# jgaeddert/liquid-usrp

Measured on AMD Instinct MI355X. Metric: complex Msamples/s through multichannelrx, higher is better.
Workload: dtype f32

## Files before the change

liquid-usrp_amd/csrc/channelizer.hip:

```cpp
#include "devel.h"
#include "devmath.h"
#include "kernels.h"
#include "sc16.hpp"
#include "devscope.hpp"

namespace mcrx {

#ifndef CH_NT_STORE
#define CH_NT_STORE 1
#endif
#ifndef CH_NT_LOAD
#define CH_NT_LOAD 1
#endif
#define CH_R 8
static_assert(MCRX_TILE_S == 2 * CH_R, "two rounds fill one granule");
#define CH_P_REF 14
#ifndef CH_RH
#define CH_RH 4
#endif
#define CH_P_OVS 28

__device__ __forceinline__ void lds_barrier()
{
    asm volatile("s_waitcnt lgkmcnt(0)\n\ts_barrier" ::: "memory");
// ... 4 lines not shown

template <int K> struct Log2 { enum { v = 1 + Log2<K / 2>::v }; };
template <> struct Log2<1> { enum { v = 0 }; };

#ifndef CH_RADIX8
#define CH_RADIX8 1
#endif
template <int K> struct Plan {
    enum { R = (CH_RADIX8 && (K == 1024 || K == 512)) ? 8 : 4, LR = R == 8 ? 3 : 2 };
    static constexpr int stages() { int L = K, s = 0; while (L > 16) { L /= R; s++; } return s; }
    static constexpr int final_size() { int L = K; while (L > 16) L /= R; return L; }
    enum { S = stages(), F = final_size(), RL = K + K / F, ROWP = RL + 1 };
};
template <int K> __device__ __forceinline__ int pad(int e) { return e + e / Plan<K>::F; }
template <int K>
__device__ __forceinline__ int dif_pos(int k)
{
    int L = K, pos = 0;
#pragma unroll
    for (int s = 0; s < Plan<K>::S; s++) { pos += (k & (Plan<K>::R - 1)) * (L >> Plan<K>::LR); k >>= Plan<K>::LR; L >>= Plan<K>::LR; }
    return pos + k;
}

__device__ __forceinline__ float2 w16(int k)
{
    const float c[8] = { 1.0f, 0.92387953251f, 0.70710678119f, 0.38268343236f, 0.0f, -0.38268343236f, -0.70710678119f, -0.92387953251f };
    const float s[8] = { 0.0f, -0.38268343236f, -0.70710678119f, -0.92387953251f, -1.0f, -0.92387953251f, -0.70710678119f, -0.38268343236f };
    return make_float2(c[k], s[k]);
}
constexpr int bitrev_c(int i, int bits) { int r = 0; for (int b = 0; b < bits; b++) if (i & (1 << b)) r |= 1 << (bits - 1 - b); return r; }

template <int F, bool LOWER = false>
__device__ __forceinline__ void fft_reg(float2 (&v)[F])
{
#pragma unroll
    for (int h = F / 2; h >= 1; h >>= 1) {
#pragma unroll
        for (int i = 0; i < F; i++) {
            if ((i & h) == 0) {
                const float2 u = v[i], w = v[i + h];
                v[i] = cadd(u, w);
                if (LOWER && h == 1) continue;
                const float2 d = csub(u, w);
                const int tk = (i & (h - 1)) * (8 / h);
                if (tk == 0) v[i + h] = d;
                else if (tk == 4) v[i + h] = cmulnj(d);
                else v[i + h] = cmul_fx(d, w16(tk));
            }
        }
    }
}

template <int K, int C, int T, int P> struct Geo {
    enum { TPS = K / C, NS = T / TPS, TILE_F2 = NS * CH_R * Plan<K>::ROWP };
    static constexpr int taps_in_lds() { const long room = (160l * 1024 - (long)TILE_F2 * 8) / (4l * K); return room >= P ? P : (int)room; }
    enum { TL = taps_in_lds() };
    static constexpr size_t lds_bytes() { return (size_t)TILE_F2 * sizeof(float2) + (size_t)TL * K * sizeof(float); }
};

template <int K, int C, int T, int P, bool SHIFT, int IN, bool EDGE>
__device__ __forceinline__ void channelizer_rounds(const ChanArgs &a, float2 *tile)
{
    typedef typename RawOf<IN>::type Raw;
    constexpr bool SC16 = IN == IQ_SC16;
    constexpr int TPS = K / C;
    constexpr int NS = T / TPS;
    constexpr int N = K / 2;
    constexpr int H = P - 1;
    constexpr int TL = Geo<K, C, T, P>::TL, TG = P - TL;
    constexpr int S = Plan<K>::S, F = Plan<K>::F, ROWP = Plan<K>::ROWP, R = Plan<K>::R, LR = Plan<K>::LR;
    static_assert(TPS * C == K && NS * TPS == T && NS >= 1, "bad channelizer geometry");
    static_assert(TL >= 1 && TG >= 0 && TG <= 8, "tap split");

    const int tid = threadIdx.x;
    const int sl = tid / TPS, cg = tid % TPS;
    const int n0 = cg * C;
    const long long slab = (long long)blockIdx.x * NS + sl;
    const long long bs = slab * (long long)a.slab_blocks;

    float *ltap = reinterpret_cast<float *>(tile + NS * CH_R * ROWP);
    {
        constexpr int NT = TL * K;
        constexpr int PER = (NT + T - 1) / T;
        float tv[PER];
#pragma unroll
        for (int i = 0; i < PER; i++) { const int idx = tid + i * T; tv[i] = a.taps[idx < NT ? idx : 0]; }
#pragma unroll
        for (int i = 0; i < PER; i++) { const int idx = tid + i * T; if (idx < NT) ltap[idx] = tv[i]; }
    }
    __syncthreads();
    float2 tw[S > 0 ? S : 1][R - 1];
#pragma unroll
    for (int st = 0; st < S; st++) {
        const int L = K >> (LR * st), q4 = L >> LR;
        const int pos = tid % q4;
#pragma unroll
        for (int r = 1; r < R; r++) {
            float sn, cs; sincos_u32((uint32_t)(r * pos) * (uint32_t)(4294967296.0 / L), sn, cs);
            tw[st][r - 1] = make_float2(cs, -sn);
        }
    }

    const uint32_t dth = a.dtheta;
    float sd1, cd1; sincos_u32(dth, sd1, cd1);
    float sk8, ck8; sincos_u32((uint32_t)K * dth, sk8, ck8);
    const uint32_t t0 = a.first_sample_lo;

    const Raw *const xin = static_cast<const Raw *>(a.x), *const hin = static_cast<const Raw *>(a.halo);
    auto load_raw = [&](long long b, Raw (&dst)[C]) {
        const Raw *src = xin + n0;
        if constexpr (EDGE) {
            const bool inx = b >= 0 && b < (long long)a.nblocks;
            const bool inh = b < 0 && hin != nullptr;
            if (inx) src = xin + (size_t)b * K + n0;
            if (inh) src = hin + (size_t)(b + H) * K + n0;
        } else if constexpr (SC16) src = xin + (uint32_t)((uint32_t)b * (uint32_t)K + (uint32_t)n0);
        else src = xin + (size_t)b * K + n0;
        if constexpr (SC16) {
            if constexpr (C == 2) {
#if CH_NT_LOAD
                typedef uint32_t v2u __attribute__((ext_vector_type(2)));
                const v2u v = __builtin_nontemporal_load(reinterpret_cast<const v2u *>(src));
#else
                const uint2 v = *reinterpret_cast<const uint2 *>(src);
#endif
                dst[0] = v.x; dst[1] = v.y;
            } else dst[0] = src[0];
        } else if constexpr (C == 2) {
#if CH_NT_LOAD
            typedef float v4f __attribute__((ext_vector_type(4)));
            const v4f v = __builtin_nontemporal_load(reinterpret_cast<const v4f *>(src));
#else
            const float4 v = *reinterpret_cast<const float4 *>(src);
#endif
            dst[0] = make_float2(v.x, v.y); dst[1] = make_float2(v.z, v.w);
        } else dst[0] = src[0];
    };
    auto osc_start = [&](long long g, float &sn, float &cs) {
        sincos_u32_hw((t0 + (uint32_t)(g * K + n0)) * dth, sn, cs);
    };
    auto osc_next_block = [&](float &sn, float &cs) {
        const float s2 = fmaf(sn, ck8, cs * sk8), c2 = fmaf(cs, ck8, -(sn * sk8)); sn = s2; cs = c2;
    };
    auto mix_with = [&](long long b, float sn, float cs, const Raw (&src)[C], float2 (&dst)[C]) {
        if constexpr (EDGE) {
            const bool valid = (b >= 0 && b < (long long)a.nblocks) || (b < 0 && a.halo != nullptr);
            sn = valid ? sn : 0.f; cs = valid ? cs : 0.f;
        }
#pragma unroll
        for (int c = 0; c < C; c++) {
            if (c > 0) { const float s2 = fmaf(sn, cd1, cs * sd1), c2 = fmaf(cs, cd1, -(sn * sd1)); sn = s2; cs = c2; }
            float x, y;
            if constexpr (SC16) { x = (float)(int16_t)(src[c] & 0xffffu) * 0x1p-15f; y = (float)((int32_t)src[c] >> 16) * 0x1p-15f; }
            else { x = src[c].x; y = src[c].y; }
            dst[c] = make_float2(fmaf(x, cs, y * sn), fmaf(y, cs, -(x * sn)));
        }
    };

    float2 s[H + CH_R][C];
    Raw w[SC16 ? H + CH_R : 1][C];
    auto raw = [&](int i) -> Raw (&)[C] { if constexpr (SC16) return w[i]; else return s[i]; };
#pragma unroll
    for (int i = 0; i < H + CH_R; i++) load_raw(bs - H + i, raw(i));
    {
        constexpr int HG = (H + CH_R - 1) / CH_R, HSKIP = HG * CH_R - H;
        static_assert(CH_R == 8, "groups of 8");
        int i = 0;
#pragma unroll
        for (int g = 0; g < HG; g++) {
            float sn, cs;
            osc_start(bs - (long long)CH_R * (HG - g), sn, cs);
#pragma unroll
            for (int k = 0; k < CH_R; k++) {
                if (g > 0 || k >= HSKIP) { mix_with(bs - H + i, sn, cs, raw(i), s[i]); i++; }
                osc_next_block(sn, cs);
            }
        }
    }

    constexpr int NBF4 = NS * CH_R * (K / R);
    constexpr int NG = NS * CH_R * (K / F);
    constexpr int NOPS = NS * N * (CH_R / 2);
    static_assert(S == 0 || (NBF4 % T == 0 && T % (K / R) == 0), "a thread's butterflies must differ by whole rows");
    static_assert(NG % T == 0 || NG < T, "F-point groups per thread");
    static_assert(NOPS % T == 0, "granule stores per thread");
    constexpr int BTRIPS = S > 0 ? NBF4 / T : 0, BSTEP = S > 0 ? (T / (K / R)) * ROWP : 0;
    int fa[S > 0 ? S : 1];
    if constexpr (S > 0) {
#pragma unroll
        for (int st = 0; st < S; st++) {
            const int L = K >> (LR * st), q4 = L >> LR;
            const int f = tid / (K / R), j = tid % (K / R);
            fa[st] = f * ROWP + pad<K>((j / q4) * L + j % q4);
        }
    }
    constexpr int GTRIPS = (NG + T - 1) / T;
    int fg[GTRIPS];
#pragma unroll
    for (int i = 0; i < GTRIPS; i++) { const int g = tid + i * T; fg[i] = (g / (K / F)) * ROWP + (g % (K / F)) * (F + 1); }
    constexpr int OTRIPS = NOPS / T;
    int ssrc[OTRIPS];
    uint32_t sdst[OTRIPS];
    int srem[OTRIPS];
#pragma unroll
    for (int k = 0; k < OTRIPS; k++) {
        const int o = tid + k * T;
        const int osl = o / (N * (CH_R / 2)), rem = o % (N * (CH_R / 2));
        const int ch = rem / (CH_R / 2), rp = rem % (CH_R / 2);
        const long long ob = ((long long)blockIdx.x * NS + osl) * (long long)a.slab_blocks;
        const int g = ch / a.cg, c = ch % a.cg;
        ssrc[k] = (osl * CH_R + 2 * rp) * ROWP + pad<K>(dif_pos<K>(ch));
        sdst[k] = (uint32_t)((((size_t)g * a.ntiles + (size_t)(ob / MCRX_TILE_S)) * a.cg + c) * (MCRX_TILE_S / 2) + rp);
        const long long left = (long long)a.nblocks - ob;
        srem[k] = left < 0 ? 0 : (left > 0x40000000ll ? 0x40000000 : (int)left);
    }
    const uint32_t tile_step = a.cg * (MCRX_TILE_S / 2);
    float4 *out4 = reinterpret_cast<float4 *>(a.out);
    int wcol[C];
#pragma unroll
    for (int c = 0; c < C; c++) wcol[c] = pad<K>(SHIFT ? (int)((n0 + c + a.col_shift) & (K - 1)) : n0 + c);

    const int rounds = a.slab_blocks / CH_R;
    for (int rd = 0; rd < rounds; rd++) {
        const long long b0 = bs + (long long)rd * CH_R;
        float tg[TG > 0 ? TG : 1][C];
#pragma unroll
        for (int j = 0; j < TG; j++)
#pragma unroll
            for (int c = 0; c < C; c++) tg[j][c] = a.taps[(size_t)(TL + j) * K + n0 + c];
        if constexpr (P <= CH_P_REF) {
            float tap[P][C];
#pragma unroll
            for (int j = 0; j < P; j++)
#pragma unroll
                for (int c = 0; c < C; c++) tap[j][c] = ltap[j * K + n0 + c];
            {
                float sn, cs;
                osc_start(b0, sn, cs);
#pragma unroll
                for (int r = 0; r < CH_R; r++) { mix_with(b0 + r, sn, cs, raw(H + r), s[H + r]); osc_next_block(sn, cs); }
            }
#pragma unroll
            for (int r = 0; r < CH_R; r++) {
                float2 v[C];
#pragma unroll
                for (int c = 0; c < C; c++) v[c] = make_float2(0.f, 0.f);
#pragma unroll
                for (int j = P - 1; j >= 0; j--) {
#pragma unroll
                    for (int c = 0; c < C; c++) {
                        v[c].x += tap[j][c] * s[H + r - j][c].x;
                        v[c].y += tap[j][c] * s[H + r - j][c].y;
                    }
                }
                float2 *row = tile + (sl * CH_R + r) * ROWP;
                if constexpr (SHIFT) {
#pragma unroll
                    for (int c = 0; c < C; c++) row[wcol[c]] = v[c];
                } else {
                    float2 *rw = row + pad<K>(n0);
#pragma unroll
                    for (int c = 0; c < C; c++) rw[c] = v[c];
                }
            }
        } else {
            {
                float sn, cs;
                osc_start(b0, sn, cs);
#pragma unroll
                for (int r = 0; r < CH_R; r++) { mix_with(b0 + r, sn, cs, raw(H + r), s[H + r]); osc_next_block(sn, cs); }
            }
#pragma unroll
            for (int rh = 0; rh < CH_R; rh += CH_RH) {
                float2 v[CH_RH][C];
#pragma unroll
                for (int r = 0; r < CH_RH; r++)
#pragma unroll
                    for (int c = 0; c < C; c++) v[r][c] = make_float2(0.f, 0.f);
#pragma unroll
                for (int j = P - 1; j >= 0; j--) {
                    float tj[C];
#pragma unroll
                    for (int c = 0; c < C; c++) tj[c] = j >= TL ? tg[j - TL][c] : ltap[j * K + n0 + c];
#pragma unroll
                    for (int r = 0; r < CH_RH; r++)
#pragma unroll
                        for (int c = 0; c < C; c++) {
                            v[r][c].x += tj[c] * s[H + rh + r - j][c].x;
                            v[r][c].y += tj[c] * s[H + rh + r - j][c].y;
                        }
                }
#pragma unroll
                for (int r = 0; r < CH_RH; r++) {
// ... 12 lines not shown
#pragma unroll
        for (int i = 0; i < H; i++)
#pragma unroll
            for (int c = 0; c < C; c++) s[i][c] = s[i + CH_R][c];
#pragma unroll
        for (int r = 0; r < CH_R; r++) load_raw(b0 + CH_R + r, raw(H + r));
        lds_barrier();

        if constexpr (S > 0) {
#pragma unroll
            for (int st = 0; st < S; st++) {
                const int L = K >> (LR * st), q4 = L >> LR;
                const int D = q4 + q4 / F;
#pragma unroll
                for (int i = 0; i < BTRIPS; i++) {
                    float2 *p = tile + fa[st] + i * BSTEP;
                    if constexpr (R == 8) {
                        float2 v[8];
#pragma unroll
                        for (int m = 0; m < 8; m++) v[m] = p[m * D];
                        fft_reg<8>(v);
                        p[0] = v[0];
#pragma unroll
                        for (int r = 1; r < 8; r++) p[r * D] = cmul_fx(v[bitrev_c(r, 3)], tw[st][r - 1]);
                        continue;
                    }
                    const float2 x0 = p[0], x1 = p[D], x2 = p[2 * D], x3 = p[3 * D];
                    const float2 a0 = cadd(x0, x2), a1 = csub(x0, x2), a2 = cadd(x1, x3), a3 = cmulnj(csub(x1, x3));
                    p[0] = cadd(a0, a2);
                    p[D] = cmul_fx(cadd(a1, a3), tw[st][0]);
                    p[2 * D] = cmul_fx(csub(a0, a2), tw[st][1]);
                    p[3 * D] = cmul_fx(csub(a1, a3), tw[st][2]);
                }
                lds_barrier();
            }
        }
        {
#pragma unroll
            for (int i = 0; i < GTRIPS; i++) {
                if (NG % T != 0 && tid + i * T >= NG) break;
                float2 *p = tile + fg[i];
                float2 v[F];
#pragma unroll
                for (int m = 0; m < F; m++) v[m] = p[m];
                fft_reg<F, (F >= 2)>(v);
#pragma unroll
                for (int m = 0; m < F; m++) if (F < 2 || bitrev_c(m, Log2<F>::v) < F / 2) p[bitrev_c(m, Log2<F>::v)] = v[m];
            }
            lds_barrier();
        }

#pragma unroll
        for (int k = 0; k < OTRIPS; k++) {
            bool ok = true;
            if constexpr (EDGE) ok = rd * CH_R < srem[k];
            if (ok) {
                const float2 *src = tile + ssrc[k];
                const float2 v0 = src[0], v1 = src[ROWP];
#if CH_NT_STORE
                { typedef float v4f __attribute__((ext_vector_type(4)));
                  v4f nv = { v0.x, v0.y, v1.x, v1.y };
                  __builtin_nontemporal_store(nv, reinterpret_cast<v4f *>(&out4[(size_t)(sdst[k] + ((uint32_t)rd >> 1) * tile_step + ((uint32_t)rd & 1u) * (CH_R / 2))])); }
#else
                out4[(size_t)(sdst[k] + ((uint32_t)rd >> 1) * tile_step + ((uint32_t)rd & 1u) * (CH_R / 2))] = make_float4(v0.x, v0.y, v1.x, v1.y);
#endif
            }
        }
        lds_barrier();
    }
}

template <int K, int C, int T, int P, bool SHIFT, int IN>
__global__ __launch_bounds__(T) void channelizer_kernel(ChanArgs a)
{
    extern __shared__ __attribute__((aligned(16))) float2 tile[];
    constexpr int NS = T / (K / C), H = P - 1;
    const long long s0 = (long long)blockIdx.x * NS;
    const long long first = s0 * (long long)a.slab_blocks - H, last = (s0 + NS) * (long long)a.slab_blocks + CH_R;
    if (first >= 0 && last <= (long long)a.nblocks) channelizer_rounds<K, C, T, P, SHIFT, IN, false>(a, tile);
    else channelizer_rounds<K, C, T, P, SHIFT, IN, true>(a, tile);
}

template <int K, int C, int T, int P, bool SHIFT, int IN>
static hipError_t launch_one(const ChanArgs &a, hipStream_t st)
{
    constexpr int NS = T / (K / C);
    const size_t lds = Geo<K, C, T, P>::lds_bytes();
    long long nslabs = ((long long)a.nblocks + a.slab_blocks - 1) / a.slab_blocks;
    unsigned grid = (unsigned)((nslabs + NS - 1) / NS);
    if (grid == 0) return hipSuccess;
    if ((unsigned long long)(K / 2) * ((unsigned long long)a.ntiles + (unsigned long long)NS * a.slab_blocks / MCRX_TILE_S + 1ull) * (MCRX_TILE_S / 2) >= (1ull << 32))
        return hipErrorInvalidValue;
    if (IN == IQ_SC16 && (unsigned long long)a.nblocks * K >= (1ull << 32)) return hipErrorInvalidValue;
    static PerDeviceOnce attr_done;
    hipError_t e = raise_lds_limit((const void *)channelizer_kernel<K, C, T, P, SHIFT, IN>, lds, attr_done);
    if (e != hipSuccess) return e;
    hipLaunchKernelGGL((channelizer_kernel<K, C, T, P, SHIFT, IN>), dim3(grid), dim3(T), lds, st, a);
    return hipGetLastError();
}

#define CG_T 256
#define CH_P CH_P_REF
#define CH_H (CH_P_REF - 1)
template <int IN> __device__ __forceinline__ float2 sample_cf32(const void *p, size_t i)
{
    if constexpr (IN == IQ_SC16) {
        return sc16_unpack(static_cast<const uint32_t *>(p)[i]);
    } else return static_cast<const float2 *>(p)[i];
}
template <int IN>
__global__ __launch_bounds__(CG_T) void channelizer_generic_kernel(ChanArgs a, uint32_t K)
{
    extern __shared__ __attribute__((aligned(16))) float2 gl[];
// ... 34 lines not shown
    const long long tl = b0 / MCRX_TILE_S; const int half = (int)((b0 / CH_R) & 1);
    for (uint32_t k = tid; k < N; k += CG_T) {
        float2 y[CH_R];
#pragma unroll
        for (int r = 0; r < CH_R; r++) y[r] = make_float2(0.f, 0.f);
        uint32_t idx = 0;
        for (uint32_t n = 0; n < K; n++) {
            const float2 w = W[idx];
#pragma unroll
            for (int r = 0; r < CH_R; r++) {
                const float2 v = V[(size_t)r * K + n];
                y[r].x += v.x * w.x - v.y * w.y; y[r].y += v.x * w.y + v.y * w.x;
            }
            idx += k; if (idx >= K) idx -= K;
        }
        const uint32_t g = k / a.cg, c = k % a.cg;
        float4 *dst = reinterpret_cast<float4 *>(a.out + (((size_t)g * a.ntiles + (size_t)tl) * a.cg + c) * MCRX_TILE_S + half * CH_R);
#pragma unroll
        for (int r = 0; r < CH_R; r += 2) dst[r / 2] = make_float4(y[r].x, y[r].y, y[r + 1].x, y[r + 1].y);
    }
}

static bool pow2_fast(unsigned K) { return K >= 2 && K <= 1024 && (K & (K - 1)) == 0; }
int channelizer_supported(unsigned K)
{ return (pow2_fast(K) || (K >= 2 && K % 2 == 0 && K <= 2048)) ? 1 : 0; }

uint32_t channelizer_auto_slab(unsigned K, size_t nblocks, unsigned ncu)
{
    const unsigned threads = K >= 1024 ? 512u : 256u, C = K >= 4 ? 2u : 1u;
    const unsigned ns = threads / (K / C > 0 ? K / C : 1u) ? threads / (K / C) : 1u;
    const size_t capacity = (size_t)ncu * (K >= 1024 ? 1u : 2u) * ns;
    const size_t k = (nblocks + capacity * 512 - 1) / (capacity * 512);
    size_t slab = (nblocks + capacity * k - 1) / (capacity * k);
    slab = (slab + MCRX_TILE_S - 1) & ~(size_t)(MCRX_TILE_S - 1);
    if (slab < 32) slab = 32;
    return (uint32_t)slab;
}

template <int IN>
static hipError_t launch_format(unsigned K, unsigned P, const ChanArgs &a, hipStream_t st)
{
    if (P == CH_P_OVS) {
        switch (K) {
        case 2:    return launch_one<2, 1, 256, CH_P_OVS, true, IN>(a, st);
        case 4:    return launch_one<4, 2, 256, CH_P_OVS, true, IN>(a, st);
        case 8:    return launch_one<8, 2, 256, CH_P_OVS, true, IN>(a, st);
        case 16:   return launch_one<16, 2, 256, CH_P_OVS, true, IN>(a, st);
        case 32:   return launch_one<32, 2, 256, CH_P_OVS, true, IN>(a, st);
        case 64:   return launch_one<64, 2, 256, CH_P_OVS, true, IN>(a, st);
        case 128:  return launch_one<128, 2, 256, CH_P_OVS, true, IN>(a, st);
        case 256:  return launch_one<256, 2, 256, CH_P_OVS, true, IN>(a, st);
        case 512:  return launch_one<512, 2, 512, CH_P_OVS, true, IN>(a, st);
        case 1024: return launch_one<1024, 2, 512, CH_P_OVS, true, IN>(a, st);
        default:   return hipErrorInvalidValue;
        }
    }
    if (P != CH_P_REF) return hipErrorInvalidValue;
    if (!pow2_fast(K)) {
        if (a.nblocks == 0) return hipSuccess;
        const size_t lds = (size_t)(CH_R + 1) * K * sizeof(float2);
        static PerDeviceOnce gen_done;
        hipError_t e = raise_lds_limit((const void *)channelizer_generic_kernel<IN>, 160 * 1024, gen_done);
        if (e != hipSuccess) return e;
        hipLaunchKernelGGL(channelizer_generic_kernel<IN>, dim3(a.nblocks / CH_R), dim3(CG_T), lds, st, a, (uint32_t)K);
        return hipGetLastError();
    }
    switch (K) {
    case 2:    return launch_one<2, 1, 256, CH_P_REF, false, IN>(a, st);
    case 4:    return launch_one<4, 2, 256, CH_P_REF, false, IN>(a, st);
    case 8:    return launch_one<8, 2, 256, CH_P_REF, false, IN>(a, st);
    case 16:   return launch_one<16, 2, 256, CH_P_REF, false, IN>(a, st);
    case 32:   return launch_one<32, 2, 256, CH_P_REF, false, IN>(a, st);
    case 64:   return launch_one<64, 2, 256, CH_P_REF, false, IN>(a, st);
    case 128:  return launch_one<128, 2, 256, CH_P_REF, false, IN>(a, st);
    case 256:  return launch_one<256, 2, 256, CH_P_REF, false, IN>(a, st);
    case 512:  return launch_one<512, 2, 256, CH_P_REF, false, IN>(a, st);
    case 1024: { static const int c1 = devel_env("MCRX_CHAN_C1") ? atoi(devel_env("MCRX_CHAN_C1")) : 0;
                 return c1 ? launch_one<1024, 1, 1024, CH_P_REF, false, IN>(a, st) : launch_one<1024, 2, 512, CH_P_REF, false, IN>(a, st); }
    default:   return hipErrorInvalidValue;
    }
}
// ... 10 lines not shown
```

liquid-usrp_amd/csrc/devmath.h:

```cpp
#pragma once
#include <hip/hip_runtime.h>
#include <stdint.h>

namespace mcrx {

typedef float2 cfd;

__device__ __forceinline__ cfd cmake(float re, float im) { return make_float2(re, im); }
__device__ __forceinline__ cfd cadd(cfd a, cfd b) { return make_float2(a.x + b.x, a.y + b.y); }
__device__ __forceinline__ cfd csub(cfd a, cfd b) { return make_float2(a.x - b.x, a.y - b.y); }
__device__ __forceinline__ cfd cmul(cfd a, cfd b)
{ return make_float2(a.x * b.x - a.y * b.y, a.x * b.y + a.y * b.x); }
__device__ __forceinline__ cfd cmul_fx(cfd a, cfd b)
{ return make_float2(fmaf(a.x, b.x, -(a.y * b.y)), fmaf(a.x, b.y, a.y * b.x)); }
__device__ __forceinline__ cfd cmulc(cfd a, cfd b)
{ return make_float2(a.x * b.x + a.y * b.y, a.y * b.x - a.x * b.y); }
__device__ __forceinline__ cfd cscale(cfd a, float g) { return make_float2(a.x * g, a.y * g); }
__device__ __forceinline__ cfd cmulnj(cfd a) { return make_float2(a.y, -a.x); }
typedef float devmath_v2f __attribute__((ext_vector_type(2)));
__device__ __forceinline__ cfd cadd_nj(cfd a, cfd b)
{
    devmath_v2f r; const devmath_v2f av = { a.x, a.y }, bv = { b.x, b.y };
    asm("v_pk_add_f32 %0, %1, %2 op_sel:[0,1] op_sel_hi:[1,0] neg_hi:[0,1]" : "=v"(r) : "v"(av), "v"(bv));
    return make_float2(r.x, r.y);
}
__device__ __forceinline__ cfd csub_nj(cfd a, cfd b)
{
    devmath_v2f r; const devmath_v2f av = { a.x, a.y }, bv = { b.x, b.y };
    asm("v_pk_add_f32 %0, %1, %2 op_sel:[0,1] op_sel_hi:[1,0] neg_lo:[0,1]" : "=v"(r) : "v"(av), "v"(bv));
    return make_float2(r.x, r.y);
}

__device__ __forceinline__ void sincos_u32(uint32_t th, float &s, float &c)
{
    uint32_t t = th + 0x20000000u;
    uint32_t q = t >> 30;
    int32_t r = (int32_t)(t & 0x3FFFFFFFu) - 0x20000000;
    float a = (float)r * 1.4629180792671596e-09f;
    float a2 = a * a;
    float sp = a + a * a2 * (-1.6666654611e-1f + a2 * (8.3321608736e-3f + a2 * (-1.9515295891e-4f)));
    float cp = 1.0f - 0.5f * a2 + a2 * a2 * (4.166664568298827e-2f + a2 * (-1.388731625493765e-3f + a2 * 2.443315711809948e-5f));
    float ss = (q & 1) ? cp : sp;
    float cc = (q & 1) ? sp : cp;
    s = (q & 2) ? -ss : ss;
    c = ((q + 1) & 2) ? -cc : cc;
}
__device__ __forceinline__ void sincos_u32_hw(uint32_t th, float &s, float &c)
{
    const float rev = (float)(int32_t)th * 2.3283064365386963e-10f;
    s = __builtin_amdgcn_sinf(rev);
    c = __builtin_amdgcn_cosf(rev);
}
__device__ __forceinline__ cfd mix_down_hw(cfd x, uint32_t th)
{
// ... 126 lines not shown
```

liquid-usrp_amd/csrc/kernels.h:

```cpp
#pragma once
#include <hip/hip_runtime.h>
#include <stdint.h>
#include "acq_shared.h"

namespace mcrx {

#define MCRX_TILE_S 16
#define MCRX_TILE_SH 4
#define MCRX_HDR_SYMS 288
#define MCRX_HDR_ENC 36
#define MCRX_HDR_DEC 14

struct ChanArgs {
    const void *x;
    const void *halo;
    const float *taps;
    float2 *out;
    uint32_t nblocks;
    uint32_t slab_blocks;
    uint32_t first_sample_lo;
    uint32_t dtheta;
    uint32_t ntiles;
    uint32_t cg;
    uint32_t col_shift;
};
int channelizer_supported(unsigned K);
uint32_t channelizer_auto_slab(unsigned K, size_t nblocks, unsigned ncu);
hipError_t channelizer_launch(unsigned K, unsigned P, unsigned in_fmt, const ChanArgs &a, hipStream_t st);

#ifndef MCRX_S1_BACKOFF_CORRECTION
#define MCRX_S1_BACKOFF_CORRECTION 0
#endif
#ifndef MCRX_S1_METRIC_G0_NORMALISED
#define MCRX_S1_METRIC_G0_NORMALISED 1
#endif
enum { SY_SEEK = 0, SY_S0A, SY_S0B, SY_S1, SY_RX };
enum { FX_HEADER = 0, FX_PAYLOAD };

struct CodingDev {
    const uint32_t *crc_byte;
    const uint32_t *crc_zadv;
    const uint8_t *qam16_nb;
    const uint8_t *qam64_nb;
};

struct SyncConsts {
    int M, M2, cp, L, backoff, M_pilot, M_data, Nen, M_S0, M_S1;
    int E;
    int log2M;
// ... 161 lines not shown
```

liquid-usrp_amd/csrc/mcrx_hip.hip:

```cpp
#include "../../include/mcrx_hip.h"
#include "acq_plan.hpp"
#include "config_read.hpp"
#include "design.hpp"
#include "devel.h"
#include "devmath.h"
#include "devscope.hpp"
#include "kernels.h"
#include "sc16.hpp"
#include "txcode.hpp"

#include <algorithm>
#include <chrono>
#include <cstdio>
#include <cstdlib>
#include <cstring>
#include <mutex>
#include <string>
#include <vector>

using namespace mcrx;

#define MCRX_SLOTS 8
#define MCRX_GENS 4

// ... 119 lines not shown
    int gen = 0; bool gen_used[MCRX_GENS] = {}, gen_closed[MCRX_GENS] = {}, gen_abandoned[MCRX_GENS] = {};
    uint32_t round_lds_pad = 0;
    uint32_t walk_lds_pad = 13312;
    int payload_fr = 1, payload_lean = 1, payload_xb = 63;
    int debug = 0, no_fast = 0, seek_burst = 1, acq_mode = 0; bool free_run = false;
    hipStream_t acq_stream = nullptr;
    uint64_t gen_close_seq[MCRX_GENS] = {}, close_counter = 0;
    hipEvent_t ev_gen[MCRX_GENS] = {};
    hipEvent_t ev_clean[MCRX_GENS] = {};
    bool clean_pending[MCRX_GENS] = {};
    uint64_t sarena_cap = 0;
    PayloadJob *d_jobs[MCRX_SLOTS] = {}; uint32_t *d_njobs = nullptr; float2 *d_jR[MCRX_SLOTS] = {};
    uint32_t *d_gen[MCRX_SLOTS] = {}, *d_qam[MCRX_SLOTS] = {}, *d_live[MCRX_SLOTS] = {};
    uint2 *d_vit_scratch = nullptr; uint32_t vit_rows = 0, vit_waves = 0, vit_mode = 0; uint32_t *d_vit_passes = nullptr;
    uint64_t seq = 0;
    unsigned nslots = 5;
    uint32_t *d_stats = nullptr;
    bool pipelined = true;
    hipStream_t s_scout = nullptr, s_work = nullptr, s_copy = nullptr;
    hipStream_t s_side = nullptr; hipEvent_t ev_side[MCRX_SLOTS] = {}, ev_side_last = nullptr; bool side_last = false;

    hipEvent_t ev_ready[MCRX_SLOTS] = {}, ev_scout[MCRX_SLOTS] = {}, ev_done[MCRX_SLOTS] = {}, ev_in = nullptr, ev_consumed = nullptr, ev_tmp[4] = {};
    int last_slot = -1; size_t last_ntiles = 0;
    uint32_t spec_stride = MCRX_SPEC_MAX;
    SpecSlot *d_spec = nullptr; float2 *d_spec_R = nullptr; int64_t *d_anchor = nullptr, *d_seekst = nullptr;
    bool spec = false;
    uint32_t *h_hint = nullptr, *d_hint = nullptr;
    uint8_t *d_jsoft[MCRX_SLOTS] = {}, *d_jtmp[MCRX_SLOTS] = {};
    bool scout = true, scout_tables = true, il_tried = false;
    bool acq_prio = true;
    AcqPolicy acq;
    int lean_build = 1;
    int seg_walker = 1;
    uint64_t total_samples = 0;
    uint64_t stage_first = 0;
    int64_t chan_samples = 0;
    uint32_t in_fmt = IQ_CF32; size_t ss = sizeof(float2);
    char *d_hist[2] = { nullptr, nullptr }; int hist_cur = 0;
    char *d_in = nullptr;
    char *h_stage = nullptr; size_t stage_cap = 0, stage_fill = 0;
    float2 *d_chan[MCRX_SLOTS] = {}; size_t chan_cap_tiles = 0;
    unsigned hist_tiles = 0; uint64_t defer = 0;
    unsigned chan_P = 14, hist_blocks = 13, col_shift = 0;
    bool oversampled = false; mcrx_hip_pfb2_t pfb2 = nullptr; const float *d_h1 = nullptr;
    float2 *d_pfin[2] = { nullptr, nullptr }, *d_pfout[2] = { nullptr, nullptr }; size_t pf_cap_blocks = 0; int pf_cur = 0;
    uint64_t pf_in_valid = 0, pf_steps = 0; size_t pf_last_blocks = 0; bool pf_have_last = false;
// ... 258 lines not shown
    a.nch = q->nch; a.nfft = m.nfft; a.window = m.window;
    a.carry_len = m.carry_len; a.carry_cap = 256;
    a.carry_in = m.d_carry[m.carry_cur]; a.carry_out = m.d_carry[m.carry_cur ^ 1];
    a.nsplit = (uint32_t)std::max<uint64_t>(1, std::min<uint64_t>(m.max_split, S / 4));
    const size_t nb = (size_t)q->nch * m.nfft;
    a.part_psd = m.d_part; a.part_level = m.d_part + (size_t)m.max_split * nb;
    a.part_peak = reinterpret_cast<float *>(a.part_level + (size_t)m.max_split * q->nch);
    a.psd = m.d_sums; a.level = m.d_sums + (size_t)q->nch * 256; a.peak = reinterpret_cast<float *>(a.level + q->nch);
    HIPCHK(monitor_launch(a, sm));
    HIPCHK(hipEventRecord(m.ev_last, sm));
    m.carry_cur ^= 1; m.carry_len = (uint32_t)(total - S * m.nfft);
    m.nseg += S; m.nsamp += (uint64_t)ntiles * MCRX_TILE; m.next = first + ntiles * MCRX_TILE;
    m.used = sm != st;
    return MCRX_OK;
}

static size_t hist_bytes(mcrx_hip_t q) { return ((size_t)q->hist_blocks * q->K * q->ss + 15) & ~(size_t)15; }

static int restart_async(mcrx_hip_t q, hipStream_t st, bool from_zero)
{
    if (from_zero) { q->total_samples = 0; q->chan_samples = 0; }
    q->stage_fill = 0; q->stage_first = q->total_samples;
    q->hist_cur = 0;
    q->last_slot = -1; q->last_ntiles = 0;
    q->pf_in_valid = 0; q->pf_steps = 0; q->pf_have_last = false;
    monitor_restart(q);
    RC(join_into(q, st));
    for (int g = 0; g < MCRX_GENS; g++) {
        HIPCHK(sync_reset_launch(q->d_st, q->nch, q->chan_samples, g == 0 ? reinterpret_cast<float2 *>(q->d_hist[0]) : nullptr,
                                 g == 0 ? reinterpret_cast<float2 *>(q->d_hist[1]) : nullptr,
                                 hist_bytes(q) / sizeof(float2), q->d_nrec[g], q->d_arena_used[g],
                                 nullptr, st));
        q->gen_used[g] = false; q->gen_closed[g] = false; q->gen_abandoned[g] = false;
    }
    if (q->d_seekst) HIPCHK(hipMemsetAsync(q->d_seekst, 0, (size_t)q->nch * 2 * sizeof(int64_t), st));
    q->gen = 0;
    RC(fork_from(q, st));
    return MCRX_OK;
}

static void read_devel_env(mcrx_hip_t q)
{
    q->debug = getenv("MCRX_DEBUG") ? atoi(getenv("MCRX_DEBUG")) : 0;
    if (devel_env("MCRX_SERIAL")) q->pipelined = false;
    q->scout = devel_env("MCRX_NO_SCOUT") == nullptr;
    if (!q->scout || devel_env("MCRX_NO_SPEC")) q->spec = false;
    if (devel_env("MCRX_NO_PRIO")) q->acq_prio = false;
// ... 237 lines not shown
        for (hipEvent_t e : { q->mon.ev_in, q->mon.ev_out, q->mon.ev_last }) if (e) (void)hipEventDestroy(e);
        if (q->mon.s_mon) (void)hipStreamDestroy(q->mon.s_mon);
    }
    if (q->copy_stream) (void)hipStreamDestroy(q->copy_stream);
    if (q->h_hint) (void)hipHostFree(q->h_hint);
    for (int w = 0; w < MCRX_NKERNELS; w++) for (auto e : q->evring[w]) if (e) (void)hipEventDestroy(e);
    if (q->stream) (void)hipStreamDestroy(q->stream);
    delete q;
    return MCRX_OK;
}

extern "C" unsigned mcrx_hip_num_channels(mcrx_hip_t q) { return q ? q->N : 0; }
extern "C" unsigned mcrx_hip_input_format(mcrx_hip_t q) { return q ? q->in_fmt : 0; }
extern "C" uint32_t mcrx_hip_nco_step(mcrx_hip_t q) { return q ? q->dtheta : 0; }
extern "C" unsigned mcrx_hip_history_blocks(mcrx_hip_t q) { return q ? q->hist_blocks : 0; }
extern "C" int mcrx_hip_get_taps(mcrx_hip_t q, float *h, size_t n)
{
    if (!q || !h || n < q->taps.size()) return fail(MCRX_EINVAL, "taps buffer too small");
    memcpy(h, q->taps.data(), q->taps.size() * sizeof(float));
    return MCRX_OK;
}

static int launch_channelizer(mcrx_hip_t q, const void *x, size_t nblocks, uint64_t first_sample,
                              const void *halo, float2 *out, unsigned groups, size_t ntiles_stride, hipStream_t st)
{
    if (nblocks == 0) return MCRX_OK;
    if (nblocks % MCRX_TILE) return fail(MCRX_EINVAL, "nblocks must be a multiple of MCRX_TILE (16)");
    if (groups == 0 || q->N % groups) return fail(MCRX_EINVAL, "groups must divide the channel count");
    ChanArgs a;
    a.x = x; a.halo = halo; a.taps = q->d_taps; a.out = out;
    a.nblocks = (uint32_t)nblocks;
    a.slab_blocks = q->slab_blocks ? q->slab_blocks : channelizer_auto_slab(q->K, nblocks, q->ncu);
    a.first_sample_lo = (uint32_t)first_sample; a.dtheta = q->dtheta;
    a.ntiles = (uint32_t)ntiles_stride; a.cg = q->N / groups; a.col_shift = q->col_shift;
    RC(q->ev_begin(0, st));
    HIPCHK(channelizer_launch(q->K, q->chan_P, q->in_fmt, a, st));
    RC(q->ev_end(0, st));
    return MCRX_OK;
}
static int sync_lazy_allocs(mcrx_hip_t q, const AcqPlan &plan)
{
    if (!q->il_tried) {
        q->il_tried = true;
        if (q->scout_tables && devel_env("MCRX_NO_ILMAP") == nullptr &&
            il_tables_acquire(q->max_payload, q->max_enc, &q->sc.il_map, &q->sc.il_off, &q->sc.il_n, q->stream) != MCRX_OK) {
            (void)hipGetLastError();
            q->sc.il_map = nullptr; q->sc.il_off = nullptr; q->sc.il_n = 0;
            if (q->debug) fprintf(stderr, "[mcrx] de-interleaver gather tables not built (%s): decoding without them\n", mcrx_hip_last_error());
        }
    }
    if (!q->d_vit_scratch && q->vit_mode == 0 && q->vit_rows && plan.want_k7) {
        const size_t vit_bytes = (size_t)q->vit_waves * q->vit_rows * 64 * sizeof(uint2);
        if (hipMalloc((void **)&q->d_vit_scratch, vit_bytes) != hipSuccess) {
            (void)hipGetLastError(); q->d_vit_scratch = nullptr; q->vit_mode = 2;
            if (q->debug) fprintf(stderr, "[mcrx] the K = 7 decoder's scratch (%zu MB) could not be allocated: the block decoder stays\n", vit_bytes >> 20);
        } else q->owned.push_back(q->d_vit_scratch);
    }
// ... 191 lines not shown
extern "C" int mcrx_hip_kernel_timing(mcrx_hip_t q, int on)
{
    if (!q) return -1;
    const int was = q->ev_on ? 1 : 0;
    q->ev_on = on != 0;
    return was;
}

static int ensure_chan(mcrx_hip_t q, size_t tiles)
{
    if (tiles <= q->chan_cap_tiles) return MCRX_OK;
    HIPCHK(hipDeviceSynchronize());
    float2 *nb[MCRX_SLOTS] = {};
    const size_t n = tiles * (size_t)q->N * MCRX_TILE, tile_elems = (size_t)q->N * MCRX_TILE;
    for (unsigned i = 0; i < q->nslots; i++) {
        HIPCHK(hipMalloc((void **)&nb[i], n * sizeof(float2)));
        HIPCHK(hipMemset(nb[i], 0, n * sizeof(float2)));
    }
    if (q->last_slot >= 0)
        HIPCHK(hipMemcpy(nb[q->last_slot] + q->last_ntiles * tile_elems, q->d_chan[q->last_slot] + q->last_ntiles * tile_elems,
                         (size_t)q->hist_tiles * tile_elems * sizeof(float2), hipMemcpyDeviceToDevice));
    for (int i = 0; i < MCRX_SLOTS; i++) { if (q->d_chan[i]) (void)hipFree(q->d_chan[i]); q->d_chan[i] = nb[i]; }
    q->chan_cap_tiles = tiles;
    return MCRX_OK;
}

static int run_oversampled(mcrx_hip_t q, const float2 *x, size_t nblocks, uint64_t first_abs, float2 *tiles, hipStream_t sc)
{
    const size_t M = q->K, N = q->N, lead = (size_t)28 * N, hsteps = 32, nsteps = 2 * nblocks, nin = nblocks * q->K;
    if (nblocks > q->pf_cap_blocks) {
        HIPCHK(hipDeviceSynchronize());
        float2 *ni[2] = { nullptr, nullptr }, *no[2] = { nullptr, nullptr };
        for (int i = 0; i < 2; i++) {
            HIPCHK(hipMalloc((void **)&ni[i], (lead + nblocks * q->K) * sizeof(float2)));
            HIPCHK(hipMalloc((void **)&no[i], (hsteps + 2 * nblocks) * M * sizeof(float2)));
            HIPCHK(hipMemset(ni[i], 0, lead * sizeof(float2)));
            HIPCHK(hipMemset(no[i], 0, hsteps * M * sizeof(float2)));
        }
        if (q->pf_have_last) {
            const int c = q->pf_cur;
            HIPCHK(hipMemcpy(ni[c] + q->pf_last_blocks * q->K, q->d_pfin[c] + q->pf_last_blocks * q->K, lead * sizeof(float2), hipMemcpyDeviceToDevice));
            HIPCHK(hipMemcpy(no[c] + 2 * q->pf_last_blocks * M, q->d_pfout[c] + 2 * q->pf_last_blocks * M, hsteps * M * sizeof(float2), hipMemcpyDeviceToDevice));
        }
        for (int i = 0; i < 2; i++) {
            if (q->d_pfin[i]) (void)hipFree(q->d_pfin[i]);
            if (q->d_pfout[i]) (void)hipFree(q->d_pfout[i]);
// ... 19 lines not shown
                       out + hsteps * M, (uint32_t)M, (uint32_t)N, (uint32_t)(nblocks / MCRX_TILE), q->d_h1, tiles);
    HIPCHK(hipGetLastError());
    RC(q->ev_end(0, sc));
    q->pf_cur = cur; q->pf_last_blocks = nblocks; q->pf_have_last = true;
    q->pf_in_valid += nin; q->pf_steps += nsteps;
    return MCRX_OK;
}

static int run_blocks(mcrx_hip_t q, const void *x, size_t nblocks, uint64_t first_abs, hipStream_t st)
{
    if (nblocks == 0) return MCRX_OK;
    if (q->chan_samples + (int64_t)nblocks >= MCRX_POSITION_MAX) return fail(MCRX_EINVAL, "channel-rate positions must stay below MCRX_POSITION_MAX = 2^48");
    const size_t ntiles = nblocks / MCRX_TILE;
    RC(ensure_chan(q, q->hist_tiles + ntiles));
    const int slot = (int)(q->seq % q->nslots);
    float2 *buf = q->d_chan[slot];
    const size_t tile_elems = (size_t)q->N * MCRX_TILE;
    hipStream_t sc = st;
    if (q->pipelined) {
        sc = q->stream;
        if (st != sc) { HIPCHK(hipEventRecord(q->ev_in, st)); HIPCHK(hipStreamWaitEvent(sc, q->ev_in, 0)); }
        if (q->seq >= q->nslots) HIPCHK(hipStreamWaitEvent(sc, q->ev_done[slot], 0));
    }
    if (q->last_slot >= 0)
        HIPCHK(hipMemcpyAsync(buf, q->d_chan[q->last_slot] + q->last_ntiles * tile_elems,
                              (size_t)q->hist_tiles * tile_elems * sizeof(float2), hipMemcpyDeviceToDevice, sc));
    if (q->bypass)
        HIPCHK(hipMemcpyAsync(buf + q->hist_tiles * tile_elems, x, nblocks * sizeof(float2), hipMemcpyDeviceToDevice, sc));
    else if (q->oversampled)
        RC(run_oversampled(q, static_cast<const float2 *>(x), nblocks, first_abs, buf + q->hist_tiles * tile_elems, sc));
    else
        RC(launch_channelizer(q, x, nblocks, first_abs, q->d_hist[q->hist_cur], buf + q->hist_tiles * tile_elems, 1, ntiles, sc));
    if (!q->bypass && !q->oversampled) {
        const uint64_t nh = (uint64_t)q->hist_blocks * q->K;
        const dim3 hg((unsigned)((nh + 255) / 256));
        if (q->in_fmt == IQ_SC16)
            hipLaunchKernelGGL(hist_update_kernel<uint32_t>, hg, dim3(256), 0, sc, reinterpret_cast<const uint32_t *>(q->d_hist[q->hist_cur]),
                               static_cast<const uint32_t *>(x), (uint64_t)nblocks * q->K, reinterpret_cast<uint32_t *>(q->d_hist[1 - q->hist_cur]), nh);
        else
            hipLaunchKernelGGL(hist_update_kernel<float2>, hg, dim3(256), 0, sc, reinterpret_cast<const float2 *>(q->d_hist[q->hist_cur]),
                               static_cast<const float2 *>(x), (uint64_t)nblocks * q->K, reinterpret_cast<float2 *>(q->d_hist[1 - q->hist_cur]), nh);
        HIPCHK(hipGetLastError());
        q->hist_cur ^= 1;
    }
    if (sc != st) {
        HIPCHK(hipEventRecord(q->ev_consumed, sc));
        HIPCHK(hipStreamWaitEvent(st, q->ev_consumed, 0));
    }
    const int64_t buf_first = q->chan_samples - (int64_t)q->hist_tiles * MCRX_TILE;
    q->last_slot = slot; q->last_ntiles = ntiles;
    RC(launch_sync(q, buf, q->N, q->ch_first, buf_first, q->chan_samples + (int64_t)nblocks, sc));
    q->chan_samples += (int64_t)nblocks;
    return MCRX_OK;
}

static int process_staged(mcrx_hip_t q)
// ... 472 lines not shown
```

Measured before the change: 188,500.

## Fuse history carry and tile copy into channelizer, use packed complex math

The channelizer kernel now writes the next call's input history (hist_out) and a second copy of the trailing tiles into the next slot (out2). This removes the separate hist_update kernel launch and the device-to-device memcpy of history tiles on the next call. It also switches the complex multiplies and oscillator rotations to packed v_pk_mul/v_pk_fma inline asm, and the twiddle sincos to a polynomial version. The cost is extra global writes inside the main kernel, an extra event wait on the next slot, and more complex state tracking for the carried data.

```diff
diff --git a/liquid-usrp_amd/csrc/channelizer.hip b/liquid-usrp_amd/csrc/channelizer.hip
--- a/liquid-usrp_amd/csrc/channelizer.hip
+++ b/liquid-usrp_amd/csrc/channelizer.hip
@@ -50,6 +50,33 @@
     return pos + k;
 }
 
+__device__ __forceinline__ void polys_semi(float a, float a2, float p1, float q1, float &sp, float &cp)
+{
+#pragma clang fp contract(off)
+    const float ps = -1.6666654611e-1f + a2 * p1, pc = 4.166664568298827e-2f + a2 * q1;
+    const float ts = (a * a2) * ps, tc = (a2 * a2) * pc;
+    sp = a + ts;
+    cp = tc + fmaf(a2, -0.5f, 1.0f);
+}
+template <bool SEMI = false>
+__device__ __forceinline__ void sincos_u32_fx(uint32_t th, float &s, float &c)
+{
+    const uint32_t t = th + 0x20000000u, q = t >> 30;
+    const int32_t r = (int32_t)(t & 0x3FFFFFFFu) - 0x20000000;
+    const float a = (float)r * 1.4629180792671596e-09f;
+    const float a2 = a * a;
+    const float p1 = fmaf(a2, -1.9515295891e-4f, 8.3321608736e-3f), q1 = fmaf(a2, 2.443315711809948e-5f, -1.388731625493765e-3f);
+    float sp, cp;
+    if constexpr (SEMI) polys_semi(a, a2, p1, q1, sp, cp);
+    else {
+        sp = fmaf(a * a2, fmaf(a2, p1, -1.6666654611e-1f), a);
+        cp = fmaf(a2 * a2, fmaf(a2, q1, 4.166664568298827e-2f), fmaf(a2, -0.5f, 1.0f));
+    }
+    const float ss = (q & 1) ? cp : sp, cc = (q & 1) ? sp : cp;
+    s = (q & 2) ? -ss : ss;
+    c = ((q + 1) & 2) ? -cc : cc;
+}
+
 __device__ __forceinline__ float2 w16(int k)
 {
     const float c[8] = { 1.0f, 0.92387953251f, 0.70710678119f, 0.38268343236f, 0.0f, -0.38268343236f, -0.70710678119f, -0.92387953251f };
@@ -73,7 +100,7 @@
                 const int tk = (i & (h - 1)) * (8 / h);
                 if (tk == 0) v[i + h] = d;
                 else if (tk == 4) v[i + h] = cmulnj(d);
-                else v[i + h] = cmul_fx(d, w16(tk));
+                else v[i + h] = cmul_fx_pk(d, w16(tk));
             }
         }
     }
@@ -96,6 +123,7 @@
     constexpr int N = K / 2;
     constexpr int H = P - 1;
     constexpr int TL = Geo<K, C, T, P>::TL, TG = P - TL;
+    constexpr bool PKM = !(P > CH_P_REF && K >= 512);
     constexpr int S = Plan<K>::S, F = Plan<K>::F, ROWP = Plan<K>::ROWP, R = Plan<K>::R, LR = Plan<K>::LR;
     static_assert(TPS * C == K && NS * TPS == T && NS >= 1, "bad channelizer geometry");
     static_assert(TL >= 1 && TG >= 0 && TG <= 8, "tap split");
@@ -107,6 +135,11 @@
     const long long bs = slab * (long long)a.slab_blocks;
 
     float *ltap = reinterpret_cast<float *>(tile + NS * CH_R * ROWP);
+    constexpr uint32_t NH = (uint32_t)H * K;
+    const bool carry_hist = a.hist_out != nullptr;
+    const Raw *const hsrc = static_cast<const Raw *>(a.x) + (carry_hist ? (size_t)(a.nblocks - H) * K : 0);
+    uint32_t hidx = blockIdx.x * T + tid;
+    Raw hval = hsrc[carry_hist ? (hidx < NH ? hidx : NH - 1) : 0];
     {
         constexpr int NT = TL * K;
         constexpr int PER = (NT + T - 1) / T;
@@ -117,6 +150,14 @@
         for (int i = 0; i < PER; i++) { const int idx = tid + i * T; if (idx < NT) ltap[idx] = tv[i]; }
     }
     __syncthreads();
+    if (carry_hist) {
+        Raw *const hdst = static_cast<Raw *>(a.hist_out);
+        while (hidx < NH) {
+            hdst[hidx] = hval;
+            hidx += gridDim.x * T;
+            if (hidx < NH) hval = hsrc[hidx];
+        }
+    }
     float2 tw[S > 0 ? S : 1][R - 1];
 #pragma unroll
     for (int st = 0; st < S; st++) {
@@ -124,14 +165,16 @@
         const int pos = tid % q4;
 #pragma unroll
         for (int r = 1; r < R; r++) {
-            float sn, cs; sincos_u32((uint32_t)(r * pos) * (uint32_t)(4294967296.0 / L), sn, cs);
+            float sn, cs;
+            if (R == 8 && r == 1) sincos_u32_fx<true>((uint32_t)(r * pos) * (uint32_t)(4294967296.0 / L), sn, cs);
+            else sincos_u32_fx((uint32_t)(r * pos) * (uint32_t)(4294967296.0 / L), sn, cs);
             tw[st][r - 1] = make_float2(cs, -sn);
         }
     }
 
     const uint32_t dth = a.dtheta;
-    float sd1, cd1; sincos_u32(dth, sd1, cd1);
-    float sk8, ck8; sincos_u32((uint32_t)K * dth, sk8, ck8);
+    float2 od1; sincos_u32_fx(dth, od1.x, od1.y);
+    float2 ok8; sincos_u32_fx((uint32_t)K * dth, ok8.x, ok8.y);
     const uint32_t t0 = a.first_sample_lo;
 
     const Raw *const xin = static_cast<const Raw *>(a.x), *const hin = static_cast<const Raw *>(a.halo);
@@ -164,24 +207,23 @@
             dst[0] = make_float2(v.x, v.y); dst[1] = make_float2(v.z, v.w);
         } else dst[0] = src[0];
     };
-    auto osc_start = [&](long long g, float &sn, float &cs) {
-        sincos_u32_hw((t0 + (uint32_t)(g * K + n0)) * dth, sn, cs);
+    auto osc_start = [&](long long g, float2 &o) {
+        sincos_u32_hw((t0 + (uint32_t)(g * K + n0)) * dth, o.x, o.y);
+        if constexpr (PKM) o = trans_settle(o);
     };
-    auto osc_next_block = [&](float &sn, float &cs) {
-        const float s2 = fmaf(sn, ck8, cs * sk8), c2 = fmaf(cs, ck8, -(sn * sk8)); sn = s2; cs = c2;
-    };
-    auto mix_with = [&](long long b, float sn, float cs, const Raw (&src)[C], float2 (&dst)[C]) {
+    auto osc_next_block = [&](float2 &o) { o = PKM ? rot_fx_pk(o, ok8) : rot_fx(o, ok8); };
+    auto mix_with = [&](long long b, float2 o, const Raw (&src)[C], float2 (&dst)[C]) {
         if constexpr (EDGE) {
             const bool valid = (b >= 0 && b < (long long)a.nblocks) || (b < 0 && a.halo != nullptr);
-            sn = valid ? sn : 0.f; cs = valid ? cs : 0.f;
+            o.x = valid ? o.x : 0.f; o.y = valid ? o.y : 0.f;
         }
 #pragma unroll
         for (int c = 0; c < C; c++) {
-            if (c > 0) { const float s2 = fmaf(sn, cd1, cs * sd1), c2 = fmaf(cs, cd1, -(sn * sd1)); sn = s2; cs = c2; }
+            if (c > 0) o = PKM ? rot_fx_pk(o, od1) : rot_fx(o, od1);
             float x, y;
             if constexpr (SC16) { x = (float)(int16_t)(src[c] & 0xffffu) * 0x1p-15f; y = (float)((int32_t)src[c] >> 16) * 0x1p-15f; }
             else { x = src[c].x; y = src[c].y; }
-            dst[c] = make_float2(fmaf(x, cs, y * sn), fmaf(y, cs, -(x * sn)));
+            dst[c] = PKM ? rot_fx_pk(make_float2(x, y), o) : rot_fx(make_float2(x, y), o);
         }
     };
 
@@ -196,12 +238,12 @@
         int i = 0;
 #pragma unroll
         for (int g = 0; g < HG; g++) {
-            float sn, cs;
-            osc_start(bs - (long long)CH_R * (HG - g), sn, cs);
+            float2 o;
+            osc_start(bs - (long long)CH_R * (HG - g), o);
 #pragma unroll
             for (int k = 0; k < CH_R; k++) {
-                if (g > 0 || k >= HSKIP) { mix_with(bs - H + i, sn, cs, raw(i), s[i]); i++; }
-                osc_next_block(sn, cs);
+                if (g > 0 || k >= HSKIP) { mix_with(bs - H + i, o, raw(i), s[i]); i++; }
+                osc_next_block(o);
             }
         }
     }
@@ -244,6 +286,7 @@
     }
     const uint32_t tile_step = a.cg * (MCRX_TILE_S / 2);
     float4 *out4 = reinterpret_cast<float4 *>(a.out);
+    const uint32_t wg_tile_end = (uint32_t)((((long long)blockIdx.x * NS + NS - 1) * (long long)a.slab_blocks) / MCRX_TILE_S) + 1u;
     int wcol[C];
 #pragma unroll
     for (int c = 0; c < C; c++) wcol[c] = pad<K>(SHIFT ? (int)((n0 + c + a.col_shift) & (K - 1)) : n0 + c);
@@ -263,10 +306,10 @@
 #pragma unroll
                 for (int c = 0; c < C; c++) tap[j][c] = ltap[j * K + n0 + c];
             {
-                float sn, cs;
-                osc_start(b0, sn, cs);
-#pragma unroll
-                for (int r = 0; r < CH_R; r++) { mix_with(b0 + r, sn, cs, raw(H + r), s[H + r]); osc_next_block(sn, cs); }
+                float2 o;
+                osc_start(b0, o);
+#pragma unroll
+                for (int r = 0; r < CH_R; r++) { mix_with(b0 + r, o, raw(H + r), s[H + r]); osc_next_block(o); }
             }
 #pragma unroll
             for (int r = 0; r < CH_R; r++) {
@@ -293,10 +336,10 @@
             }
         } else {
             {
-                float sn, cs;
-                osc_start(b0, sn, cs);
-#pragma unroll
-                for (int r = 0; r < CH_R; r++) { mix_with(b0 + r, sn, cs, raw(H + r), s[H + r]); osc_next_block(sn, cs); }
+                float2 o;
+                osc_start(b0, o);
+#pragma unroll
+                for (int r = 0; r < CH_R; r++) { mix_with(b0 + r, o, raw(H + r), s[H + r]); osc_next_block(o); }
             }
 #pragma unroll
             for (int rh = 0; rh < CH_R; rh += CH_RH) {
@@ -355,15 +398,15 @@
                         fft_reg<8>(v);
                         p[0] = v[0];
 #pragma unroll
-                        for (int r = 1; r < 8; r++) p[r * D] = cmul_fx(v[bitrev_c(r, 3)], tw[st][r - 1]);
+                        for (int r = 1; r < 8; r++) p[r * D] = cmul_fx_pk(v[bitrev_c(r, 3)], tw[st][r - 1]);
                         continue;
                     }
                     const float2 x0 = p[0], x1 = p[D], x2 = p[2 * D], x3 = p[3 * D];
                     const float2 a0 = cadd(x0, x2), a1 = csub(x0, x2), a2 = cadd(x1, x3), a3 = cmulnj(csub(x1, x3));
                     p[0] = cadd(a0, a2);
-                    p[D] = cmul_fx(cadd(a1, a3), tw[st][0]);
-                    p[2 * D] = cmul_fx(csub(a0, a2), tw[st][1]);
-                    p[3 * D] = cmul_fx(csub(a1, a3), tw[st][2]);
+                    p[D] = cmul_fx_pk(cadd(a1, a3), tw[st][0]);
+                    p[2 * D] = cmul_fx_pk(csub(a0, a2), tw[st][1]);
+                    p[3 * D] = cmul_fx_pk(csub(a1, a3), tw[st][2]);
                 }
                 lds_barrier();
             }
@@ -399,6 +442,20 @@
 #endif
             }
         }
+        if (__builtin_expect(a.out2 != nullptr && (wg_tile_end + ((uint32_t)rd >> 1)) * tile_step > a.out2_first, 0)) {
+            float4 *out24 = reinterpret_cast<float4 *>(a.out2);
+#pragma unroll
+            for (int k = 0; k < OTRIPS; k++) {
+                const uint32_t dst = sdst[k] + ((uint32_t)rd >> 1) * tile_step + ((uint32_t)rd & 1u) * (CH_R / 2);
+                bool ok = dst >= a.out2_first;
+                if constexpr (EDGE) ok = ok && rd * CH_R < srem[k];
+                if (ok) {
+                    const float2 *src = tile + ssrc[k];
+                    const float2 v0 = src[0], v1 = src[ROWP];
+                    out24[(size_t)(dst - a.out2_first)] = make_float4(v0.x, v0.y, v1.x, v1.y);
+                }
+            }
+        }
         lds_barrier();
     }
 }
@@ -422,6 +479,7 @@
     long long nslabs = ((long long)a.nblocks + a.slab_blocks - 1) / a.slab_blocks;
     unsigned grid = (unsigned)((nslabs + NS - 1) / NS);
     if (grid == 0) return hipSuccess;
+    if (a.hist_out != nullptr && a.nblocks < (uint32_t)(P - 1)) return hipErrorInvalidValue;
     if ((unsigned long long)(K / 2) * ((unsigned long long)a.ntiles + (unsigned long long)NS * a.slab_blocks / MCRX_TILE_S + 1ull) * (MCRX_TILE_S / 2) >= (1ull << 32))
         return hipErrorInvalidValue;
     if (IN == IQ_SC16 && (unsigned long long)a.nblocks * K >= (1ull << 32)) return hipErrorInvalidValue;
@@ -502,6 +560,7 @@
 }
 
 static bool pow2_fast(unsigned K) { return K >= 2 && K <= 1024 && (K & (K - 1)) == 0; }
+int channelizer_carries(unsigned K) { return pow2_fast(K) ? 1 : 0; }
 int channelizer_supported(unsigned K)
 { return (pow2_fast(K) || (K >= 2 && K % 2 == 0 && K <= 2048)) ? 1 : 0; }
 
@@ -537,6 +596,7 @@
     }
     if (P != CH_P_REF) return hipErrorInvalidValue;
     if (!pow2_fast(K)) {
+        if (a.out2 != nullptr || a.hist_out != nullptr) return hipErrorInvalidValue;
         if (a.nblocks == 0) return hipSuccess;
         const size_t lds = (size_t)(CH_R + 1) * K * sizeof(float2);
         static PerDeviceOnce gen_done;
diff --git a/liquid-usrp_amd/csrc/devmath.h b/liquid-usrp_amd/csrc/devmath.h
--- a/liquid-usrp_amd/csrc/devmath.h
+++ b/liquid-usrp_amd/csrc/devmath.h
@@ -30,6 +30,29 @@
     asm("v_pk_add_f32 %0, %1, %2 op_sel:[0,1] op_sel_hi:[1,0] neg_lo:[0,1]" : "=v"(r) : "v"(av), "v"(bv));
     return make_float2(r.x, r.y);
 }
+__device__ __forceinline__ cfd cmul_fx_pk(cfd a, cfd b)
+{
+    devmath_v2f t, r; const devmath_v2f av = { a.x, a.y }, bv = { b.x, b.y };
+    asm("v_pk_mul_f32 %0, %1, %2 op_sel:[1,1] op_sel_hi:[1,0] neg_lo:[1,0]" : "=v"(t) : "v"(av), "v"(bv));
+    asm("v_pk_fma_f32 %0, %1, %2, %3 op_sel_hi:[0,1,1]" : "=v"(r) : "v"(av), "v"(bv), "v"(t));
+    return make_float2(r.x, r.y);
+}
+__device__ __forceinline__ cfd rot_fx(cfd v, cfd o)
+{ return make_float2(fmaf(v.x, o.y, v.y * o.x), fmaf(v.y, o.y, -(v.x * o.x))); }
+__device__ __forceinline__ cfd rot_fx_pk(cfd v, cfd o)
+{
+    devmath_v2f t, r; const devmath_v2f vv = { v.x, v.y }, ov = { o.x, o.y };
+    asm("v_pk_mul_f32 %0, %1, %2 op_sel:[1,0] op_sel_hi:[0,0] neg_hi:[1,0]" : "=v"(t) : "v"(vv), "v"(ov));
+    asm("v_pk_fma_f32 %0, %1, %2, %3 op_sel:[0,1,0] op_sel_hi:[1,1,1]" : "=v"(r) : "v"(vv), "v"(ov), "v"(t));
+    return make_float2(r.x, r.y);
+}
+
+__device__ __forceinline__ cfd trans_settle(cfd v)
+{
+    devmath_v2f vv = { v.x, v.y };
+    asm("s_nop 0" : "+v"(vv));
+    return make_float2(vv.x, vv.y);
+}
 
 __device__ __forceinline__ void sincos_u32(uint32_t th, float &s, float &c)
 {
diff --git a/liquid-usrp_amd/csrc/kernels.h b/liquid-usrp_amd/csrc/kernels.h
--- a/liquid-usrp_amd/csrc/kernels.h
+++ b/liquid-usrp_amd/csrc/kernels.h
@@ -23,8 +23,12 @@
     uint32_t ntiles;
     uint32_t cg;
     uint32_t col_shift;
+    float2 *out2;
+    uint32_t out2_first;
+    void *hist_out;
 };
 int channelizer_supported(unsigned K);
+int channelizer_carries(unsigned K);
 uint32_t channelizer_auto_slab(unsigned K, size_t nblocks, unsigned ncu);
 hipError_t channelizer_launch(unsigned K, unsigned P, unsigned in_fmt, const ChanArgs &a, hipStream_t st);
 
diff --git a/liquid-usrp_amd/csrc/mcrx_hip.hip b/liquid-usrp_amd/csrc/mcrx_hip.hip
--- a/liquid-usrp_amd/csrc/mcrx_hip.hip
+++ b/liquid-usrp_amd/csrc/mcrx_hip.hip
@@ -165,6 +165,7 @@
 
     hipEvent_t ev_ready[MCRX_SLOTS] = {}, ev_scout[MCRX_SLOTS] = {}, ev_done[MCRX_SLOTS] = {}, ev_in = nullptr, ev_consumed = nullptr, ev_tmp[4] = {};
     int last_slot = -1; size_t last_ntiles = 0;
+    bool carried = false; uint64_t carried_seq = 0;
     uint32_t spec_stride = MCRX_SPEC_MAX;
     SpecSlot *d_spec = nullptr; float2 *d_spec_R = nullptr; int64_t *d_anchor = nullptr, *d_seekst = nullptr;
     bool spec = false;
@@ -469,7 +470,7 @@
     if (from_zero) { q->total_samples = 0; q->chan_samples = 0; }
     q->stage_fill = 0; q->stage_first = q->total_samples;
     q->hist_cur = 0;
-    q->last_slot = -1; q->last_ntiles = 0;
+    q->last_slot = -1; q->last_ntiles = 0; q->carried = false;
     q->pf_in_valid = 0; q->pf_steps = 0; q->pf_have_last = false;
     monitor_restart(q);
     RC(join_into(q, st));
@@ -753,7 +754,8 @@
 }
 
 static int launch_channelizer(mcrx_hip_t q, const void *x, size_t nblocks, uint64_t first_sample,
-                              const void *halo, float2 *out, unsigned groups, size_t ntiles_stride, hipStream_t st)
+                              const void *halo, float2 *out, unsigned groups, size_t ntiles_stride, hipStream_t st,
+                              float2 *out2 = nullptr, size_t out2_first_tile = 0, void *hist_out = nullptr)
 {
     if (nblocks == 0) return MCRX_OK;
     if (nblocks % MCRX_TILE) return fail(MCRX_EINVAL, "nblocks must be a multiple of MCRX_TILE (16)");
@@ -764,6 +766,8 @@
     a.slab_blocks = q->slab_blocks ? q->slab_blocks : channelizer_auto_slab(q->K, nblocks, q->ncu);
     a.first_sample_lo = (uint32_t)first_sample; a.dtheta = q->dtheta;
     a.ntiles = (uint32_t)ntiles_stride; a.cg = q->N / groups; a.col_shift = q->col_shift;
+    if (out2 && groups != 1) return fail(MCRX_EINVAL, "a second copy of the last tiles needs a one-group launch");
+    a.out2 = out2; a.out2_first = (uint32_t)(out2_first_tile * a.cg * (MCRX_TILE / 2)); a.hist_out = hist_out;
     RC(q->ev_begin(0, st));
     HIPCHK(channelizer_launch(q->K, q->chan_P, q->in_fmt, a, st));
     RC(q->ev_end(0, st));
@@ -1001,6 +1005,7 @@
                          (size_t)q->hist_tiles * tile_elems * sizeof(float2), hipMemcpyDeviceToDevice));
     for (int i = 0; i < MCRX_SLOTS; i++) { if (q->d_chan[i]) (void)hipFree(q->d_chan[i]); q->d_chan[i] = nb[i]; }
     q->chan_cap_tiles = tiles;
+    q->carried = false;
     return MCRX_OK;
 }
 
@@ -1066,7 +1071,12 @@
         if (st != sc) { HIPCHK(hipEventRecord(q->ev_in, st)); HIPCHK(hipStreamWaitEvent(sc, q->ev_in, 0)); }
         if (q->seq >= q->nslots) HIPCHK(hipStreamWaitEvent(sc, q->ev_done[slot], 0));
     }
-    if (q->last_slot >= 0)
+    const bool direct = !q->bypass && !q->oversampled && channelizer_carries(q->K);
+    const unsigned next = (unsigned)((q->seq + 1) % q->nslots);
+    const bool carry_tiles = direct && q->pipelined && q->nslots >= 4 && ntiles >= q->hist_tiles;
+    const bool carry_hist = direct && nblocks >= q->hist_blocks;
+    if (carry_tiles && q->seq + 1 >= q->nslots) HIPCHK(hipStreamWaitEvent(sc, q->ev_done[next], 0));
+    if (q->last_slot >= 0 && !(q->carried && q->carried_seq == q->seq))
         HIPCHK(hipMemcpyAsync(buf, q->d_chan[q->last_slot] + q->last_ntiles * tile_elems,
                               (size_t)q->hist_tiles * tile_elems * sizeof(float2), hipMemcpyDeviceToDevice, sc));
     if (q->bypass)
@@ -1074,8 +1084,11 @@
     else if (q->oversampled)
         RC(run_oversampled(q, static_cast<const float2 *>(x), nblocks, first_abs, buf + q->hist_tiles * tile_elems, sc));
     else
-        RC(launch_channelizer(q, x, nblocks, first_abs, q->d_hist[q->hist_cur], buf + q->hist_tiles * tile_elems, 1, ntiles, sc));
-    if (!q->bypass && !q->oversampled) {
+        RC(launch_channelizer(q, x, nblocks, first_abs, q->d_hist[q->hist_cur], buf + q->hist_tiles * tile_elems, 1, ntiles, sc,
+                              carry_tiles ? q->d_chan[next] : nullptr, ntiles - (carry_tiles ? q->hist_tiles : 0), carry_hist ? q->d_hist[1 - q->hist_cur] : nullptr));
+    q->carried = carry_tiles; q->carried_seq = q->seq + 1;
+    if (carry_hist) q->hist_cur ^= 1;
+    else if (!q->bypass && !q->oversampled) {
         const uint64_t nh = (uint64_t)q->hist_blocks * q->K;
         const dim3 hg((unsigned)((nh + 255) / 256));
         if (q->in_fmt == IQ_SC16)
```

Result: faster. 190,600, median of 6 (+1.1%).
